# yuanqing-wang/stag

Hardware: AMD Instinct MI355X
Metric: aggregated edges/sec, stochastic-aggregation layer-forward, ogbn-arxiv-shaped CSR (higher is better)
Workload: dtype f32

## Files before the change

stag_amd/csrc/agg_kernel.hpp:

```cpp
#pragma once
#include "../../include/stag_hip.h"
#include "noise.hpp"
#include "entry_args.hpp"
#include <stdlib.h>

namespace stag {

struct AggArgs {
  const int32_t* indptr;
  const int32_t* indices;
  const int32_t* eid;
  const int32_t* nidx;
  int32_t n_rows;
  const float* x;
  int64_t ldx;
  int32_t D;
  uint32_t ldxb;
  uint32_t ldwb;
  uint32_t x_bytes;
  int32_t wide;
  const float* p0;
  const float* p1;
  float p0s, p1s;
  int32_t pmode;
  int32_t nflags, in_norm;
  int32_t wgroup;
  PhiloxKey key;
  uint32_t pos_lo, pos_hi;
  uint32_t chunk_base;
  int32_t n_heavy;
  int32_t n_heavy_blocks;
  struct alignas(32) Walk {
    int32_t smask, sshift;
    int32_t jh_heavy;
    int32_t jh_light;
    int32_t sh;
    int32_t lbase;
    int32_t sl;
    int32_t n_total;
  } walk;
  const int32_t* xcd;
  const float* src_scale;
  const float* dst_scale;
  int32_t mean;
  float* out;
  float* outx[3];
  int32_t mc;
  uint64_t mc_stride;
  int64_t ldo;
  float* norm_scale_out;
  const float* xown;
  int64_t ldxo;
  const float* own_scale;
  float* eg0;
  float* eg1;
  float* dp_part;
  const stag_unit* units;
  const stag_unit* units_plan;
  int32_t n_units;
  const int32_t* long_rows;
  const int32_t* long_seg_ptr;
  int32_t n_long;
  int32_t n_seg;
  int32_t* seg_counters;
  float* ws;
  int32_t ws_stride;
  uint32_t ws_bytes;
  uint32_t idx_bytes;
};

__device__ __forceinline__ void load4(const float* p, int k0, int D, bool vec, float (&v)[4]) {
  if (vec) {
    const float4 t = *reinterpret_cast<const float4*>(p + k0);
    v[0] = t.x; v[1] = t.y; v[2] = t.z; v[3] = t.w;
  } else {
#pragma unroll
    for (int j = 0; j < 4; ++j) v[j] = (k0 + j < D) ? p[k0 + j] : 0.0f;
  }
}

__device__ __forceinline__ void store4(float* p, int k0, int D, bool vec, const float (&v)[4]) {
  if (vec) {
    *reinterpret_cast<float4*>(p + k0) = make_float4(v[0], v[1], v[2], v[3]);
  } else {
#pragma unroll
    for (int j = 0; j < 4; ++j)
      if (k0 + j < D) p[k0 + j] = v[j];
  }
}

__device__ __forceinline__ void store4_sc1(__amdgpu_buffer_rsrc_t rsrc, uint32_t off, int k0, int D,
                                           bool vec, const float (&v)[4]) {
  typedef unsigned int u32x4 __attribute__((ext_vector_type(4)));
  if (vec) {
    const u32x4 t = {__float_as_uint(v[0]), __float_as_uint(v[1]), __float_as_uint(v[2]),
                     __float_as_uint(v[3])};
    __builtin_amdgcn_raw_buffer_store_b128(t, rsrc, (int)off, 0, 16);
  } else {
#pragma unroll
    for (int j = 0; j < 4; ++j)
      if (k0 + j < D)
        __builtin_amdgcn_raw_buffer_store_b32(__float_as_uint(v[j]), rsrc, (int)(off + 4u * j), 0, 16);
  }
}

template <int NF, bool VEC>
__device__ __forceinline__ void kahan_sum_partials(const float* ws, int ws_stride, int s0, int s1,
                                                   int k0, int D, float (&sum)[4], float (&comp)[4]) {
  comp[0] = comp[1] = comp[2] = comp[3] = 0.f;
  sum[0] = sum[1] = sum[2] = sum[3] = 0.f;
#pragma unroll 1
  for (int s = s0; s < s1; s += NF) {
    float t[NF][4];
#pragma unroll
    for (int i = 0; i < NF; ++i) {
      if (s + i < s1) load4(ws + (int64_t)(s + i) * ws_stride, k0, D, VEC, t[i]);
      else t[i][0] = t[i][1] = t[i][2] = t[i][3] = 0.f;
    }
#pragma unroll
    for (int i = 0; i < NF; ++i)
#pragma unroll
      for (int q = 0; q < 4; ++q) {
        const float y = t[i][q] - comp[q];
        const float n = sum[q] + y;
        comp[q] = (n - sum[q]) - y;
        sum[q] = n;
      }
  }
}

__device__ __forceinline__ void agg_epilogue_extra(const AggArgs& a, float* out, int v, int deg, int k0,
                                                   bool vec, float (&acc)[4]);

constexpr int kCombineGroup = 16;
template <int NF, bool VEC, int LPE, int SLOTS>
__device__ __forceinline__ void two_level_sum(const float* ws, int ws_stride, int s0, int s1, int k0,
                                              int D, int sl, int slot0, float (&sum)[4]) {
  float comp[4] = {0.f, 0.f, 0.f, 0.f};
  sum[0] = sum[1] = sum[2] = sum[3] = 0.f;
#pragma unroll 1
  for (int g0 = s0; g0 < s1; g0 += kCombineGroup * SLOTS) {
    const int gs = g0 + sl * kCombineGroup;
    float gsum[4] = {0.f, 0.f, 0.f, 0.f}, gres[4] = {0.f, 0.f, 0.f, 0.f};
    if (gs < s1) {
      const int ge = min(gs + kCombineGroup, s1);
      kahan_sum_partials<NF, VEC>(ws, ws_stride, gs, ge, k0, D, gsum, gres);
    }
#pragma unroll
    for (int j = 0; j < SLOTS; ++j) {
      if (g0 + j * kCombineGroup < s1) {
#pragma unroll
        for (int q = 0; q < 4; ++q) {
          const float gj = SLOTS > 1 ? __int_as_float(__builtin_amdgcn_ds_bpermute(
                                           slot0 + j * (LPE << 2), __float_as_int(gsum[q])))
                                     : gsum[q];
          const float rj = SLOTS > 1 ? __int_as_float(__builtin_amdgcn_ds_bpermute(
                                           slot0 + j * (LPE << 2), __float_as_int(gres[q])))
                                     : gres[q];
          comp[q] += rj;
          const float y = gj - comp[q];
          const float n = sum[q] + y;
          comp[q] = (n - sum[q]) - y;
          sum[q] = n;
        }
      }
    }
  }
#pragma unroll
  for (int q = 0; q < 4; ++q) sum[q] -= comp[q];
}

__device__ __forceinline__ void agg_epilogue_to(const AggArgs& a, float* out, float* norm_scale_out, int v, int deg,
                                                int k0, bool vec, float (&acc)[4], const float (&wsum)[4]);
__device__ __forceinline__ void agg_epilogue(const AggArgs& a, int v, int deg, int k0, bool vec,
                                             float (&acc)[4], const float (&wsum)[4]) {
  agg_epilogue_to(a, a.out, a.norm_scale_out, v, deg, k0, vec, acc, wsum);
}
__device__ __forceinline__ void agg_epilogue_to(const AggArgs& a, float* out, float* norm_scale_out, int v, int deg,
                                                int k0, bool vec, float (&acc)[4], const float (&wsum)[4]) {
  float dv = a.dst_scale ? a.dst_scale[v] : 1.0f;
  if (a.mean) dv *= __builtin_amdgcn_rcpf((float)(deg > 1 ? deg : 1));
  if (a.in_norm) {
    float s[4];
#pragma unroll
    for (int j = 0; j < 4; ++j) {
      s[j] = (wsum[j] != 0.0f) ? (float)deg / wsum[j] : 1.0f;
      acc[j] *= s[j];
    }
    if (norm_scale_out) store4(norm_scale_out + (int64_t)v * a.D, k0, a.D, vec, s);
  }
  if (!out) return;
#pragma unroll
  for (int j = 0; j < 4; ++j) acc[j] *= dv;
  store4(out + (int64_t)v * a.ldo, k0, a.D, vec, acc);
}

__device__ __forceinline__ void agg_epilogue_extra(const AggArgs& a, float* out, int v, int deg, int k0,
                                                   bool vec, float (&acc)[4]) {
  float dv = a.dst_scale ? a.dst_scale[v] : 1.0f;
  if (a.mean) dv *= __builtin_amdgcn_rcpf((float)(deg > 1 ? deg : 1));
#pragma unroll
  for (int j = 0; j < 4; ++j) acc[j] *= dv;
  store4(out + (int64_t)v * a.ldo, k0, a.D, vec, acc);
}

__device__ __forceinline__ const float* row_at(const float* base, int idx, uint32_t stride_bytes,
                                               uint32_t koff, bool wide) {
  const char* b = reinterpret_cast<const char*>(base);
  if (wide) return reinterpret_cast<const float*>(b + (uint64_t)(uint32_t)idx * stride_bytes + koff);
  return reinterpret_cast<const float*>(b + (__umul24((uint32_t)idx, stride_bytes) + koff));
}

typedef unsigned int u32x4_t __attribute__((ext_vector_type(4)));
__device__ __forceinline__ void bufrow4(__amdgpu_buffer_rsrc_t rsrc, int idx, uint32_t stride_bytes,
                                        uint32_t koff, float (&v)[4]) {
#ifndef STAG_X_AUX
#define STAG_X_AUX 0
#endif
  const u32x4_t t = __builtin_amdgcn_raw_buffer_load_b128(
      rsrc, (int)(__umul24((uint32_t)idx, stride_bytes) + koff), 0, STAG_X_AUX);
  v[0] = __uint_as_float(t.x); v[1] = __uint_as_float(t.y);
  v[2] = __uint_as_float(t.z); v[3] = __uint_as_float(t.w);
}

__device__ __forceinline__ void loadrow4(const float* p, int k0, int D, bool vec, float (&v)[4]) {
  if (vec) {
    const float4 t = *reinterpret_cast<const float4*>(p);
    v[0] = t.x; v[1] = t.y; v[2] = t.z; v[3] = t.w;
  } else {
#pragma unroll
    for (int j = 0; j < 4; ++j) v[j] = (k0 + j < D) ? p[j] : 0.0f;
  }
}

#ifndef STAG_KAHAN_MIN_LEN
#define STAG_KAHAN_MIN_LEN 16
#endif
constexpr int kKahanMinLen = STAG_KAHAN_MIN_LEN;

#ifndef STAG_BLK_RNG
#define STAG_BLK_RNG 2
#endif
#ifndef STAG_BLK_MEM
#define STAG_BLK_MEM 2
#endif
#ifndef STAG_WAVES_PER_SIMD
#define STAG_WAVES_PER_SIMD 1
#endif
#ifndef STAG_BLOCK_THREADS
#define STAG_BLOCK_THREADS 256
#endif
#ifndef STAG_LOAD_PRIO
#define STAG_LOAD_PRIO 1
#endif
#ifndef STAG_PRIO_MIN_LEN
#define STAG_PRIO_MIN_LEN 24
// ... 498 lines not shown
      __builtin_amdgcn_s_setprio(3);
#endif
      T.fetch_idx(I, p0);
      T.pin_idx(I);
      T.fetch_rows(R, I, p0);
#if STAG_LOAD_PRIO
      if (len > STAG_PRIO_MIN_LEN) __builtin_amdgcn_s_setprio(2); else __builtin_amdgcn_s_setprio(0);
#endif
      T.compute(R, I, p0);
    }
    }
  }

#ifdef STAG_TRACE
  if (trace) trace[1] = wall_clock64();
#endif
  if constexpr (PEDGE == 4) {
#pragma unroll
    for (int i = 0; i < 2; ++i)
#pragma unroll
      for (int q = 0; q < 4; ++q) dp_out[i][q] = T.DP.v[i][q];
  }
  if (slot < 0) {
    if (sl != 0) return;
    agg_epilogue(a, v, len, k0, VEC, T.acc, T.wsum);
    if constexpr (NOUT > 1) {
#pragma unroll
      for (int o = 0; o < NOUT - 1; ++o) {
        if constexpr (WN) agg_epilogue_to(a, a.outx[o], nullptr, v, len, k0, VEC, T.X.acc[o], T.XW.w[o]);
        else agg_epilogue_extra(a, a.outx[o], v, len, k0, VEC, T.X.acc[o]);
      }
    }
#ifdef STAG_TRACE
    if (trace) trace[3] = wall_clock64();
#endif
    return;
  }
  const int r = v;
  const __amdgpu_buffer_rsrc_t rws = __builtin_amdgcn_make_buffer_rsrc(a.ws, 0, (int)a.ws_bytes, 0x00020000);
  const uint32_t woff = (uint32_t)slot * ((uint32_t)a.ws_stride * 4u) + (uint32_t)k0 * 4u;
  if (sl == 0) {
    store4_sc1(rws, woff, k0, a.D, VEC, T.acc);
    if (PEDGE != 3 && PEDGE != 4 && a.in_norm) store4_sc1(rws, woff + (uint32_t)(NOUT * a.D) * 4u, k0, a.D, VEC, T.wsum);
    if constexpr (NOUT > 1) {
#pragma unroll
      for (int o = 0; o < NOUT - 1; ++o) {
        store4_sc1(rws, woff + (uint32_t)(o + 1) * (uint32_t)a.D * 4u, k0, a.D, VEC, T.X.acc[o]);
        if constexpr (WN) store4_sc1(rws, woff + (uint32_t)(NOUT + o + 1) * (uint32_t)a.D * 4u, k0, a.D, VEC, T.XW.w[o]);
      }
    }
  }
  const int s0 = a.long_seg_ptr[r], s1 = a.long_seg_ptr[r + 1];
  asm volatile("s_waitcnt vmcnt(0)" ::: "memory");
  int ticket = 0;
  int32_t* counter = a.seg_counters + (int64_t)blockIdx.y * a.n_long + r;
  if (c == 0 && sl == 0)
    ticket = __hip_atomic_fetch_add(counter, 1, __ATOMIC_RELAXED, __HIP_MEMORY_SCOPE_AGENT);
  const int lane0 = ((int)(threadIdx.x & 63) - c - sl * LPE) << 2;
  ticket = __builtin_amdgcn_ds_bpermute(lane0, ticket);
#ifdef STAG_TRACE
  if (trace) trace[2] = wall_clock64();
#endif
  if (ticket != (s1 - s0) - 1) return;
  __builtin_amdgcn_fence(__ATOMIC_ACQUIRE, "agent");
  asm volatile("s_waitcnt vmcnt(0)" ::: "memory");
  if (c == 0 && sl == 0) *counter = 0;
  const int row = a.long_rows[r];
  const int deg = a.indptr[row + 1] - a.indptr[row];
#ifndef STAG_COMBINE_NF
#define STAG_COMBINE_NF 8
#endif
  constexpr int NF = STAG_COMBINE_NF;
  float facc[4], fws[4] = {0.f, 0.f, 0.f, 0.f};
  const int slot0 = lane0 + (c << 2);
  two_level_sum<NF, VEC, LPE, SLOTS>(a.ws, a.ws_stride, s0, s1, k0, a.D, sl, slot0, facc);
  if (PEDGE != 3 && PEDGE != 4 && a.in_norm) two_level_sum<NF, VEC, LPE, SLOTS>(a.ws + NOUT * a.D, a.ws_stride, s0, s1, k0, a.D, sl, slot0, fws);
  if (sl != 0) return;
  agg_epilogue(a, row, deg, k0, VEC, facc, fws);
#pragma unroll
  for (int o = 0; o < NOUT - 1; ++o) {
    two_level_sum<NF, VEC, LPE, SLOTS>(a.ws + (o + 1) * a.D, a.ws_stride, s0, s1, k0, a.D, sl, slot0, facc);
    if constexpr (WN) {
      two_level_sum<NF, VEC, LPE, SLOTS>(a.ws + (NOUT + o + 1) * a.D, a.ws_stride, s0, s1, k0, a.D, sl, slot0, fws);
      agg_epilogue_to(a, a.outx[o], nullptr, row, deg, k0, VEC, facc, fws);
    } else {
      agg_epilogue_extra(a, a.outx[o], row, deg, k0, VEC, facc);
    }
  }
#ifdef STAG_TRACE
  if (trace) trace[3] = wall_clock64();
#endif
}

template <int KIND, int LPE>
constexpr int mult_of() {
  constexpr bool RNG = KIND >= kNormal;
  return LPE <= 4 ? (RNG ? STAG_MULT_LPE4 : 2 * STAG_MULT_LPE4)
         : LPE == 8 ? (RNG ? STAG_MULT_LPE8 : 4 * STAG_MULT_LPE8)
         : LPE == 16 ? (RNG ? STAG_MULT_LPE16 : 2 * STAG_MULT_LPE16)
                     : STAG_MULT_WIDE;
}
#ifndef STAG_HSLOTS_LPE4
#define STAG_HSLOTS_LPE4 4
#endif
#ifndef STAG_HSLOTS_LPE8
#define STAG_HSLOTS_LPE8 4
#endif
#ifndef STAG_HSLOTS_LPE16
#define STAG_HSLOTS_LPE16 2
#endif
#ifndef STAG_HSLOTS_LPE32
// ... 107 lines not shown
#ifndef STAG_MULT_WALK_WIDE
#define STAG_MULT_WALK_WIDE 2
#endif
    constexpr int MULT_W = NOUT != 1 ? 1 : (KIND == kNone && PEDGE == 0 && LPE >= 64) ? STAG_MULT_WALK_WIDE : mult_of<KIND, LPE>();
    agg_unit<KIND, LPE, VEC, PEDGE, 1, MULT_W, NOUT, MC, WN, true>(a, unit, c, 0);
  }
}

template <int KIND, int LPE, bool VEC>
__global__ __launch_bounds__(STAG_BLOCK_THREADS, STAG_WAVES_PER_SIMD) void agg_dp_kernel(const AggArgs a) {
  constexpr int TEAMS = STAG_BLOCK_THREADS / LPE;
  __shared__ float s_dp[TEAMS][2][LPE * 4];
  const int c = threadIdx.x % LPE, tm = threadIdx.x / LPE;
  const int unit = blockIdx.x * TEAMS + tm;
  float dp[2][4] = {{0.f, 0.f, 0.f, 0.f}, {0.f, 0.f, 0.f, 0.f}};
  if (unit < a.n_units) agg_unit<KIND, LPE, VEC, 4, 1, 1>(a, unit, c, 0, dp);
#pragma unroll
  for (int i = 0; i < 2; ++i)
#pragma unroll
    for (int q = 0; q < 4; ++q) s_dp[tm][i][c * 4 + q] = dp[i][q];
  __syncthreads();
  float* part = a.dp_part + ((int64_t)blockIdx.y * gridDim.x + blockIdx.x) * (2 * LPE * 4);
  for (int i = threadIdx.x; i < 2 * LPE * 4; i += STAG_BLOCK_THREADS) {
    float sum = 0.f;
#pragma unroll
    for (int j = 0; j < TEAMS; ++j) sum += s_dp[j][i / (LPE * 4)][i % (LPE * 4)];
    part[i] = sum;
  }
}

template <int KIND>
hipError_t agg_launch(const AggArgs& a, bool vec, hipStream_t stream);

#ifndef STAG_XCD_PLANLESS
#define STAG_XCD_PLANLESS 1
#endif
#ifndef STAG_AGG_LDS_BYTES
#define STAG_AGG_LDS_BYTES 0
#endif
inline bool plain_launch_ok(const AggArgs& a, bool vec, int pedge) {
  return vec && pedge == 0 && a.pmode == STAG_PARAM_SCALAR && !a.outx[0] && !a.dp_part && !a.mc && a.out &&
         !a.src_scale && !a.in_norm && !a.nidx && (a.nflags & ~(kFlagRelu | kFlagLogScale)) == 0 &&
         (a.wide & 1) == 0 && a.x_bytes != 0 && a.idx_bytes != 0;
}

template <int KIND>
void agg_launch_plain(const AggArgs& a, int lpe, bool walk, dim3 grid, hipStream_t s);

inline bool plain_enabled() {
#if defined(STAG_TRACE) || defined(STAG_EXP_NO_ROWS)
  return false;
#endif
  const char* e = getenv("STAG_AGG_PLAIN");
  return !(e && e[0] == '0' && e[1] == 0);
}

template <int KIND>
inline void agg_launch_small(const AggArgs& a_in, bool vec, int tiles, hipStream_t s) {
  AggArgs a = a_in;
  constexpr int LPE = 32, TPB = STAG_BLOCK_THREADS / LPE, TPBH = STAG_BLOCK_THREADS / (LPE * heavy_slots_of<KIND, LPE, true>());
  a.n_heavy_blocks = (a.n_heavy + TPBH - 1) / TPBH;
  const dim3 grid(a.n_heavy_blocks + (a.n_units - a.n_heavy + TPB - 1) / TPB, tiles), block(STAG_BLOCK_THREADS);
  if (grid.x == 0) return;
  if (vec) hipLaunchKernelGGL((agg_kernel<KIND, LPE, true, 0, 1, false, false, false, true>), grid, block, STAG_AGG_LDS_BYTES, s, a);
  else     hipLaunchKernelGGL((agg_kernel<KIND, LPE, false, 0, 1, false, false, false, true>), grid, block, STAG_AGG_LDS_BYTES, s, a);
}

template <int KIND, int LPE>
inline void agg_launch_shape(const AggArgs& a_in, bool vec, int pedge, int tiles, hipStream_t s) {
  if constexpr (LPE == 32 && heavy_slots_of<KIND, 32, true>() != heavy_slots_of<KIND, 32, false>()) {
    if (!a_in.outx[0] && !a_in.dp_part && pedge == 0 && !a_in.xcd && a_in.units && a_in.n_heavy > 0 &&
        a_in.n_units <= STAG_SMALL_UNITS) {
      agg_launch_small<KIND>(a_in, vec, tiles, s);
      return;
    }
  }
  AggArgs a = a_in;
  constexpr int TPB = STAG_BLOCK_THREADS / LPE;
  constexpr int HS = heavy_slots_of<KIND, LPE>();
  constexpr int TPBH = STAG_BLOCK_THREADS / (LPE * HS);
  const bool slotted = !(HS == 1 || a.outx[0] || pedge == 3 || a.dp_part);
  if (!slotted) a.n_heavy = 0;
  const bool plain = !a.outx[0] && !a.dp_part && pedge == 0;
  if (a.xcd && a.dp_part) { a.xcd = nullptr; a.units = a.units_plan; }
  a.n_heavy_blocks = (a.n_heavy + TPBH - 1) / TPBH;
  dim3 grid(a.n_heavy_blocks + (a.n_units - a.n_heavy + TPB - 1) / TPB, tiles);
  bool walk = false;
  AggArgs::Walk& w = a.walk;
  if (a.xcd) {
    walk = true;
    w.smask = STAG_XCD_STRIPES - 1; w.sshift = 3;
    w.jh_heavy = slotted ? (w.sh + TPBH - 1) / TPBH : 0;
    w.jh_light = slotted ? 0 : (w.sh + TPB - 1) / TPB;
    w.lbase = STAG_XCD_STRIPES * w.sh;
    w.n_total = STAG_XCD_STRIPES * (w.sh + w.sl);
    grid.x = STAG_XCD_STRIPES * (w.jh_heavy + w.jh_light + (w.sl + TPB - 1) / TPB);
  } else if (STAG_XCD_PLANLESS && !a.dp_part && !a.units && a.n_units >= STAG_XCD_STRIPES * TPB && a.n_units < (1 << 30)) {
    walk = true;
    w = AggArgs::Walk{STAG_XCD_STRIPES - 1, 3, 0, 0, 0, 0, 0, a.n_units};
    w.sl = ((a.n_units + STAG_XCD_STRIPES - 1) / STAG_XCD_STRIPES + TPB - 1) / TPB * TPB;
    grid.x = STAG_XCD_STRIPES * (w.sl / TPB);
  } else if (!plain && !a.dp_part) {
    walk = true;
    w = AggArgs::Walk{0, 0, 0, 0, a.n_heavy, a.n_heavy, a.n_units - a.n_heavy, a.n_units};
    w.jh_heavy = slotted ? a.n_heavy_blocks : 0;
    w.jh_light = slotted ? 0 : (w.sh + TPB - 1) / TPB;
// ... 15 lines not shown
    if (a.mc && a.outx[0]) {
      if (vec) hipLaunchKernelGGL((agg_kernel<KIND, LPE, true, 0, 2, true, false, true>), grid, block, STAG_AGG_LDS_BYTES, s, a);
      else     hipLaunchKernelGGL((agg_kernel<KIND, LPE, false, 0, 2, true, false, true>), grid, block, STAG_AGG_LDS_BYTES, s, a);
      return;
    }
  }
  if constexpr (KIND == kNormal || KIND == kUniform) {
    if (a.outx[0]) {
      if (vec) hipLaunchKernelGGL((agg_kernel<KIND, LPE, true, 0, 3, false, false, true>), grid, block, STAG_AGG_LDS_BYTES, s, a);
      else     hipLaunchKernelGGL((agg_kernel<KIND, LPE, false, 0, 3, false, false, true>), grid, block, STAG_AGG_LDS_BYTES, s, a);
      return;
    }
  }
  if constexpr (KIND == kNormal || KIND == kUniform) {
    if (a.dp_part) {
      if (vec) hipLaunchKernelGGL((agg_dp_kernel<KIND, LPE, true>), grid, block, STAG_AGG_LDS_BYTES, s, a);
      else     hipLaunchKernelGGL((agg_dp_kernel<KIND, LPE, false>), grid, block, STAG_AGG_LDS_BYTES, s, a);
      return;
    }
    if (pedge == 3) {
      if (vec) hipLaunchKernelGGL((agg_kernel<KIND, LPE, true, 3, 1, false, false, true>), grid, block, STAG_AGG_LDS_BYTES, s, a);
      else     hipLaunchKernelGGL((agg_kernel<KIND, LPE, false, 3, 1, false, false, true>), grid, block, STAG_AGG_LDS_BYTES, s, a);
      return;
    }
  }
  if constexpr (KIND >= kNormal) {
    if (pedge == 1) {
      if (vec) hipLaunchKernelGGL((agg_kernel<KIND, LPE, true, 1, 1, false, false, true>), grid, block, STAG_AGG_LDS_BYTES, s, a);
      else     hipLaunchKernelGGL((agg_kernel<KIND, LPE, false, 1, 1, false, false, true>), grid, block, STAG_AGG_LDS_BYTES, s, a);
      return;
    }
    if (pedge == 2) {
      if (vec) hipLaunchKernelGGL((agg_kernel<KIND, LPE, true, 2, 1, false, false, true>), grid, block, STAG_AGG_LDS_BYTES, s, a);
      else     hipLaunchKernelGGL((agg_kernel<KIND, LPE, false, 2, 1, false, false, true>), grid, block, STAG_AGG_LDS_BYTES, s, a);
      return;
    }
  }
  if constexpr (KIND >= kNormal && (LPE == 32 || LPE == 64)) {
    if (plain_launch_ok(a, vec, pedge) && plain_enabled()) {
      agg_launch_plain<KIND>(a, LPE, walk, grid, s);
      return;
    }
  }
  if (walk) {
    if (vec) hipLaunchKernelGGL((agg_kernel<KIND, LPE, true, 0, 1, false, false, true>), grid, block, STAG_AGG_LDS_BYTES, s, a);
    else     hipLaunchKernelGGL((agg_kernel<KIND, LPE, false, 0, 1, false, false, true>), grid, block, STAG_AGG_LDS_BYTES, s, a);
    return;
  }
  if (vec) hipLaunchKernelGGL((agg_kernel<KIND, LPE, true, 0>), grid, block, STAG_AGG_LDS_BYTES, s, a);
  else     hipLaunchKernelGGL((agg_kernel<KIND, LPE, false, 0>), grid, block, STAG_AGG_LDS_BYTES, s, a);
}

template <int KIND>
inline hipError_t agg_launch_impl(const AggArgs& a, bool vec, hipStream_t s) {
  const int nchunk = (a.D + 3) / 4;
  const int pedge = (KIND < kNormal) ? 0 : a.pmode == STAG_PARAM_PER_EDGE1 ? (a.eg0 ? 3 : 1)
                    : a.pmode == STAG_PARAM_PER_EDGE ? 2 : 0;
  const int lpe = lanes_for(nchunk, 1);
  const int tiles = (nchunk + lpe - 1) / lpe;
  switch (lpe) {
    case 64: agg_launch_shape<KIND, 64>(a, vec, pedge, tiles, s); break;
    case 32: agg_launch_shape<KIND, 32>(a, vec, pedge, tiles, s); break;
    case 16: agg_launch_shape<KIND, 16>(a, vec, pedge, tiles, s); break;
    case 8:  agg_launch_shape<KIND, 8>(a, vec, pedge, tiles, s); break;
    case 4:  agg_launch_shape<KIND, 4>(a, vec, pedge, tiles, s); break;
    case 2:  agg_launch_shape<KIND, 2>(a, vec, pedge, tiles, s); break;
    default: agg_launch_shape<KIND, 1>(a, vec, pedge, tiles, s); break;
  }
  return hipGetLastError();
}

}
```

stag_amd/csrc/api.hip:

```cpp
#include <algorithm>
#include <cmath>
#include <cstring>
#include <vector>

#include "../../include/stag_hip.h"
#include "agg_kernel.hpp"
#include "agg_max.hpp"
#include "entry_args.hpp"

using namespace stag;

namespace stag {
template <int KIND>
hipError_t agg_launch(const AggArgs& a, bool vec, hipStream_t stream);
}

namespace {

__global__ void philox_raw_kernel(PhiloxKey key, int64_t pos0, int64_t n_pos, int n_chunk,
                                  uint32_t* out) {
  const int64_t i = (int64_t)blockIdx.x * blockDim.x + threadIdx.x;
  if (i >= n_pos * n_chunk) return;
  uint32_t r[4];
  philox_at(pos0 + i / n_chunk, (uint32_t)(i % n_chunk), key, r);
// ... 765 lines not shown
    for (int f = 0; f < fine; ++f) {
      const int32_t lo = start[(size_t)x * fine + f], hi = start[(size_t)x * fine + f + 1];
      int32_t first = lo, edges = 0, units = 0;
      for (int32_t p = lo; p < hi; ++p) {
        const int32_t len = units_host[order[p]].len;
        if (units > 0 && (edges + len > max_edges || units == max_units)) {
          batches[x].emplace_back(first, units);
          first = p; edges = 0; units = 0;
        }
        edges += len; ++units;
      }
      if (units > 0) batches[x].emplace_back(first, units);
    }
  size_t per = 0;
  for (auto& b : batches) per = std::max(per, b.size());
  const int64_t nb = (int64_t)per * STAG_XCD_STRIPES;
  if (nb > 0x7FFFFFFFll) return STAG_EINVAL;
  *n_blocks_out = (int32_t)nb;
  if (!units_out_host) return STAG_OK;
  int32_t at = 0;
  block_ptr_host[0] = 0;
  for (size_t j = 0; j < per; ++j)
    for (int x = 0; x < STAG_XCD_STRIPES; ++x) {
      if (j < batches[x].size())
        for (int32_t p = 0; p < batches[x][j].second; ++p) units_out_host[at++] = units_host[order[(size_t)batches[x][j].first + p]];
      block_ptr_host[j * STAG_XCD_STRIPES + x + 1] = at;
    }
  return STAG_OK;
}
}
}

int stag_plan_blocks_xcd(const stag_unit* units_host, int32_t n_units, int64_t n_edges, int32_t fine, int32_t max_edges,
                         int32_t max_units, stag_unit* units_out_host, int32_t* block_ptr_host, int32_t* n_blocks_out) {
  if (n_units < 0 || n_edges < 0 || fine < 1 || fine > STAG_XCD_FINE_MAX || max_edges <= 0 || max_units <= 0 ||
      !n_blocks_out || (n_units > 0 && !units_host) || ((units_out_host == nullptr) != (block_ptr_host == nullptr)))
    return STAG_EINVAL;
  return plan_blocks_xcd_impl(units_host, n_units, fine, XcdKeyByPosition{n_edges > 0 ? n_edges : 1, STAG_XCD_STRIPES * fine},
                              max_edges, max_units, units_out_host, block_ptr_host, n_blocks_out);
}

int stag_plan_blocks_xcd_ranges(const stag_unit* units_host, int32_t n_units, const int64_t* cuts_host,
                                const int32_t* keys_host, int32_t n_ranges, int32_t fine, int32_t max_edges, int32_t max_units,
                                stag_unit* units_out_host, int32_t* block_ptr_host, int32_t* n_blocks_out) {
  if (n_units < 0 || fine < 1 || fine > STAG_XCD_FINE_MAX || max_edges <= 0 || max_units <= 0 || !n_blocks_out ||
      (n_units > 0 && !units_host) || ((units_out_host == nullptr) != (block_ptr_host == nullptr)) ||
      !xcd_ranges_ok(cuts_host, keys_host, n_ranges, fine)) return STAG_EINVAL;
  return plan_blocks_xcd_impl(units_host, n_units, fine, XcdKeyByRange{cuts_host, keys_host, n_ranges}, max_edges, max_units,
                              units_out_host, block_ptr_host, n_blocks_out);
}

size_t stag_plan_workspace_bytes(int32_t n_seg, int32_t D, int32_t in_norm) {
  if (n_seg <= 0 || D <= 0) return 0;
  return (size_t)n_seg * (size_t)D * (in_norm ? 2u : 1u) * sizeof(float);
}

int stag_philox_raw(uint64_t seed, uint64_t offset, int64_t pos0, int64_t n_pos, int32_t n_chunk,
                    uint32_t* out, void* stream) {
  if (!out || n_pos < 0 || n_chunk <= 0 || !aligned16(out)) return STAG_EINVAL;
  const int64_t n = n_pos * n_chunk;
  if (n == 0) return STAG_OK;
  hipLaunchKernelGGL(philox_raw_kernel, dim3((unsigned)((n + 255) / 256)), dim3(256), 0,
                     (hipStream_t)stream, make_key(seed, offset, nullptr), pos0, n_pos, n_chunk, out);
  return hipGetLastError() == hipSuccess ? STAG_OK : STAG_EIO;
}

int stag_normal_tables(float* rad, float* cosv, float* sinv, void* stream) {
  if (!rad || !cosv || !sinv) return STAG_EINVAL;
  hipLaunchKernelGGL(normal_tables_kernel, dim3((1u << 23) / 256), dim3(256), 0, (hipStream_t)stream, rad, cosv, sinv);
  return hipGetLastError() == hipSuccess ? STAG_OK : STAG_EIO;
}

struct EdgeGradOut {
  const float* xown;
  int64_t ldxo;
  float* eg0;
  float* eg1;
  float* dp_part;
};
static int agg_common(const stag_csr* csr, const stag_plan* plan, const float* x, int64_t ldx,
                      int32_t D, const stag_noise_spec* spec, int32_t reduce, const float* src_scale,
                      const float* dst_scale, float* out, int64_t ldo, float* norm_scale_out,
                      int nout, float* const* extra, int mc, uint64_t mc_stride, void* stream,
                      const EdgeGradOut* eg = nullptr) {
  int rc = check_csr(csr);
  if (rc) return rc;
  rc = check_spec(spec, csr->n_edges, D);
  if (rc) return rc;
  if (D <= 0 || (ldx != 0 && ldx < D) || ldo < D) return STAG_EINVAL;
  if (reduce != STAG_REDUCE_SUM && reduce != STAG_REDUCE_MEAN) return STAG_EINVAL;
  if (csr->n_dst == 0) return STAG_OK;
  if (!out && !norm_scale_out && !eg) return STAG_EINVAL;
  if (csr->n_edges > 0 && !x) return STAG_EINVAL;

  AggArgs a{};
  a.indptr = csr->indptr; a.indices = csr->indices; a.eid = csr->eid; a.nidx = csr->nidx;
  a.n_rows = csr->n_dst;
  a.x = x; a.ldx = ldx; a.D = D;
  a.ldxb = (uint32_t)(ldx * 4); a.ldwb = (uint32_t)D * 4u;
  {
    const uint64_t xbytes = (uint64_t)csr->n_src * (uint64_t)ldx * 4u;
    const uint64_t wbytes = (uint64_t)csr->n_edges * (uint64_t)D * 4u;
    const bool x_narrow = xbytes < (1ull << 32) && csr->n_src < (1 << 24) && (uint64_t)ldx * 4u < (1u << 24);
    const bool w_narrow = wbytes < (1ull << 32) && csr->n_edges < (1 << 24) && (uint64_t)D * 4u < (1u << 24);
    a.wide = (x_narrow ? 0 : 1) | (w_narrow ? 0 : 2);
    a.x_bytes = x_narrow ? (uint32_t)(ldx == 0 ? (uint64_t)D * 4u : xbytes) : 0u;
    a.idx_bytes = csr->n_edges < (1 << 30) ? (uint32_t)csr->n_edges * 4u : 0u;
  }
  fill_spec(a, spec, spec->deriv);
  a.in_norm = spec->in_norm;
  a.wgroup = (spec->kind == STAG_NOISE_EXPLICIT && spec->group > 1) ? spec->group : 1;
  if (a.wgroup > 1 && (D % a.wgroup != 0 || spec->in_norm)) return STAG_EINVAL;
  rc = check_positions(spec, csr->n_edges, D, spec->kind >= STAG_NOISE_NORMAL);
  if (rc) return rc;
  a.src_scale = src_scale; a.dst_scale = dst_scale; a.mean = (reduce == STAG_REDUCE_MEAN);
  a.out = out; a.ldo = ldo; a.norm_scale_out = norm_scale_out;
  for (int o = 0; o + 1 < nout; ++o) a.outx[o] = extra[o];
  a.mc = mc; a.mc_stride = mc_stride;
  if (eg) {
    a.xown = eg->xown; a.ldxo = eg->ldxo; a.own_scale = dst_scale; a.eg0 = eg->eg0; a.eg1 = eg->eg1;
    a.dp_part = eg->dp_part;
  }

  const bool use_plan = plan_in_use(plan);
  const bool has_segs = use_plan && plan->n_seg > 0;
  const bool xcd = use_plan && plan->xcd_order && !(eg && eg->dp_part);
  const size_t need = has_segs ? stag_plan_workspace_bytes(plan->n_seg, nout * D, spec->in_norm) : 0;
  rc = check_plan(plan, kPlanHeavy | (xcd ? kPlanXcd : 0) | kPlanSegPtr | kPlanWorkspace | kPlanNarrow | kPlanCounters, need);
  if (rc) return rc;
  fill_plan(a, csr, plan);
  if (use_plan) {
    a.units_plan = plan->units;
    a.n_heavy = plan->n_heavy;
    if (xcd) {
      a.xcd = plan->xcd_order;
      a.units = xcd_units(plan);
      a.walk.sh = plan->xcd_stride_heavy;
      a.walk.sl = plan->xcd_stride_light;
    }
  }
  if (has_segs) {
    a.ws_stride = D * nout * (spec->in_norm ? 2 : 1); a.ws_bytes = (uint32_t)need;
    a.seg_counters = plan->seg_counters; a.n_seg = plan->n_seg;
  }

  bool vec = (D % 4 == 0) && (ldx % 4 == 0) && (ldo % 4 == 0) && aligned16(x) && (!out || aligned16(out));
  if (norm_scale_out) vec = vec && aligned16(norm_scale_out);
  for (int o = 0; o + 1 < nout; ++o) vec = vec && aligned16(extra[o]);
  if (spec->kind == STAG_NOISE_EXPLICIT) vec = vec && aligned16(spec->p0);
  if (spec->kind >= STAG_NOISE_NORMAL && spec->param_mode != STAG_PARAM_SCALAR &&
      spec->param_mode != STAG_PARAM_PER_EDGE1)
    vec = vec && aligned16(spec->p0) && (!spec->p1 || aligned16(spec->p1));
  if (has_segs) vec = vec && aligned16(plan->workspace);
  if (eg && eg->xown) vec = vec && aligned16(eg->xown) && (eg->ldxo % 4 == 0);

  hipStream_t s = (hipStream_t)stream;
  auto launch = [&](const AggArgs& args) -> hipError_t {
    switch (spec->kind) {
      case STAG_NOISE_NONE: return agg_launch<kNone>(args, vec, s);
      case STAG_NOISE_EXPLICIT: return agg_launch<kExplicit>(args, vec, s);
      case STAG_NOISE_NORMAL: return agg_launch<kNormal>(args, vec, s);
      case STAG_NOISE_UNIFORM: return agg_launch<kUniform>(args, vec, s);
      default: return agg_launch<kBernoulli>(args, vec, s);
    }
  };
  if (launch(a) != hipSuccess) return STAG_EIO;
  return STAG_OK;
}

int stag_agg_fwd(const stag_csr* csr, const stag_plan* plan, const float* x, int64_t ldx,
                 int32_t D, const stag_noise_spec* spec, int32_t reduce, const float* src_scale,
                 const float* dst_scale, float* out, int64_t ldo, float* norm_scale_out,
                 void* stream) {
  return agg_common(csr, plan, x, ldx, D, spec, reduce, src_scale, dst_scale, out, ldo, norm_scale_out,
                    1, nullptr, 0, 0, stream);
}

int stag_agg_fwd_mc(const stag_csr* csr, const stag_plan* plan, const float* x, int64_t ldx,
                    int32_t D, const stag_noise_spec* spec, int32_t n_samples, int64_t offset_stride,
                    int32_t reduce, const float* src_scale, const float* dst_scale, float* out,
                    int64_t ldo, int64_t sample_stride, void* stream) {
  if (!spec || n_samples < 1 || offset_stride < 0 || !out) return STAG_EINVAL;
  if (spec->kind < STAG_NOISE_NORMAL || spec->deriv) return STAG_EINVAL;
  if (spec->param_mode != STAG_PARAM_SCALAR && spec->param_mode != STAG_PARAM_PER_CHANNEL) return STAG_EINVAL;
  if (n_samples > 1 && sample_stride < (int64_t)(csr ? csr->n_dst : 0) * ldo) return STAG_EINVAL;
  stag_noise_spec sp = *spec;
  const int kmax = spec->in_norm ? 2 : 4;
  for (int32_t s0 = 0; s0 < n_samples;) {
    const int k = (n_samples - s0 >= 4 && kmax >= 4) ? 4 : (n_samples - s0 >= 2) ? 2 : 1;
    sp.offset = spec->offset + (uint64_t)s0 * (uint64_t)offset_stride;
    float* extra[3] = {nullptr, nullptr, nullptr};
    for (int o = 1; o < k; ++o) extra[o - 1] = out + (int64_t)(s0 + o) * sample_stride;
    const int rc = agg_common(csr, plan, x, ldx, D, &sp, reduce, src_scale, dst_scale,
                              out + (int64_t)s0 * sample_stride, ldo, nullptr, k, extra, k > 1 ? 1 : 0,
                              (uint64_t)offset_stride, stream);
    if (rc) return rc;
// ... 425 lines not shown
```

stag_amd/ops.py:

```python
import ctypes as C

import torch

from . import _lib, _torch_ext
from .graph import DEFAULT_SEG_LEN
from .noise import EdgeNoise
from .random import _MASK64

_REDUCE = {"sum": _lib.REDUCE_SUM, "mean": _lib.REDUCE_MEAN}


def _owner(graph):
    return graph._cache_owner() if hasattr(graph, "_cache_owner") else graph


def _f32c(t):
    if t is None:
        return None
    if t.dtype != torch.float32:
        t = t.float()
    return t.contiguous()


def _none_spec():
    if _torch_ext.available():
        return _NONE_ARGS
    s = _lib.NoiseSpec()
    s.kind = _lib.NOISE_NONE
    return s


def _explicit_spec(w, relu=False, in_norm=False, group=0):
    if _torch_ext.available():
        return ([_lib.NOISE_EXPLICIT, 0, int(relu), int(in_norm), 0, int(group), 0, 0], [0, 0, 0], [0.0, 0.0], w, None, None)
    s = _lib.NoiseSpec()
    s.kind = _lib.NOISE_EXPLICIT
    s.p0 = w.data_ptr()
    s.relu, s.in_norm, s.group = int(relu), int(in_norm), int(group)
    return s


def _noise_spec(noise, in_norm=None):
    if _torch_ext.available():
        return noise.torch_args(in_norm=in_norm)
    s = noise.spec()
    if in_norm is not None:
        s.in_norm = int(in_norm)
    return s


def _targs_or_c(spec):
    return _targs_to_ctypes(spec) if isinstance(spec, tuple) else spec


def _spec_in_norm(spec):
    return bool(spec[0][3]) if isinstance(spec, tuple) else bool(spec.in_norm)


def _plan_struct(csrv, seg_len, tiles, nbytes, dev, plan_t=None, width=None, gat_width=None, drawn=False):
    if plan_t is None:
        plan_t = csrv.plan(seg_len)
    if plan_t is None:
        return None, None
    ws = torch.empty(nbytes // 4, dtype=torch.float32, device=dev) if nbytes else None
    key = (tiles, _lib.stream_of(dev))
    counters = plan_t["counters"].get(key)
    if counters is None:
        counters = torch.zeros(max(plan_t["n_long"], 1) * tiles, dtype=torch.int32, device=dev)
        plan_t["counters"][key] = counters
    order, strides, fine = csrv.xcd_order(plan_t, width, drawn) if width and plan_t.get("xcd_on") else (None, (0, 0), 0)
    units, block_ptr, n_blocks = plan_t["units"], plan_t["block_ptr"], plan_t["n_blocks"]
    if gat_width and plan_t.get("xcd_on"):
        blocks = csrv.gat_blocks(plan_t, gat_width)
        if blocks is not None:
            units, block_ptr, n_blocks, fine = blocks[0], blocks[1], blocks[2], -blocks[3]
            order = units
    plan_c = plan_t.setdefault("_structs", {}).get(key + (fine,))
    if plan_c is None:
        plan_c = _lib.Plan(plan_t["seg_len"], plan_t["n_units"], plan_t["n_long"], plan_t["n_seg"],
                           _lib.ptr(units), _lib.ptr(plan_t["long_rows"]),
                           _lib.ptr(plan_t["long_seg_ptr"]), _lib.ptr(counters), None, 0,
                           plan_t["n_heavy"] if units is plan_t["units"] else 0, n_blocks, _lib.ptr(block_ptr),
                           _lib.ptr(order), *strides)
        plan_t["_structs"][key + (fine,)] = plan_c
    plan_c.workspace, plan_c.workspace_bytes = _lib.ptr(ws), nbytes
    return plan_c, (ws, counters)


_NONE_ARGS = ([_lib.NOISE_NONE, 0, 0, 0, 0, 0, 0, 0], [0, 0, 0], [0.0, 0.0], None, None, None)


def _plan_args(csrv, plan_t, tiles, dev, width=None, drawn=False):
    if plan_t is None:
        return (None, None, None, None, None, None, [0, 0, 0, 0, 0, 0, 0, 0])
    key = (tiles, _lib.stream_of(dev))
    counters = plan_t["counters"].get(key)
    if counters is None:
        counters = torch.zeros(max(plan_t["n_long"], 1) * tiles, dtype=torch.int32, device=dev)
        plan_t["counters"][key] = counters
    order, strides, _ = csrv.xcd_order(plan_t, width, drawn) if width and plan_t.get("xcd_on") else (None, (0, 0), 0)
    ints = [plan_t["seg_len"], plan_t["n_units"], plan_t["n_long"], plan_t["n_seg"], plan_t["n_heavy"], plan_t["n_blocks"],
            *strides]
    return (plan_t["units"], plan_t["long_rows"], plan_t["long_seg_ptr"], plan_t["block_ptr"], order, counters, ints)


def _agg_fwd_torch(csrv, x, noise_args, reduce, src_scale, dst_scale, seg_len, want_norm_scale, broadcast_x):
    dev = _lib.require_device(x, csrv.indptr, src_scale, dst_scale)
    D = x.numel() if broadcast_x else x.shape[1]
    plan_t = csrv.plan(seg_len)
    out, ns = torch.ops.stag.agg_fwd(*csrv.torch_args(), *_plan_args(csrv, plan_t, (D + 255) // 256, dev, width=D,
                                                                     drawn=noise_args[0][0] >= _lib.NOISE_NORMAL), x,
                                     broadcast_x, *noise_args, reduce, src_scale, dst_scale, want_norm_scale)
    return out, (ns if want_norm_scale else None)


def _agg_raw(csrv, x, D, spec, reduce, src_scale, dst_scale, seg_len, want_norm_scale=False,
             broadcast_x=False, out=None, plan_t=None, ns_out=None):
    if isinstance(spec, tuple):
        if out is None and plan_t is None:
            return _agg_fwd_torch(csrv, x, spec, reduce, src_scale, dst_scale, seg_len, want_norm_scale, broadcast_x)
        spec = _targs_to_ctypes(spec)
    dev = _lib.require_device(x, csrv.indptr, src_scale, dst_scale)
    if out is None:
        out = torch.empty((csrv.n_dst, D), dtype=torch.float32, device=dev)
    ns = ns_out if ns_out is not None else (
        torch.empty((csrv.n_dst, D), dtype=torch.float32, device=dev) if want_norm_scale else None)
    if csrv.n_dst == 0:
        return out, ns
    if plan_t is None:
        plan_t = csrv.plan(seg_len)
    nbytes = (_lib.lib().stag_plan_workspace_bytes(plan_t["n_seg"], D, int(spec.in_norm))
              if plan_t is not None else 0)
    plan_c, _keep = _plan_struct(csrv, seg_len, (D + 255) // 256, nbytes, dev, plan_t, width=D,
                                 drawn=spec.kind >= _lib.NOISE_NORMAL)
    cs = csrv.struct()
    with _lib.on_device(dev):
        rc = _lib.lib().stag_agg_fwd(
            C.byref(cs), C.byref(plan_c) if plan_c is not None else None, _lib.ptr(x),
            0 if broadcast_x else x.stride(0), D, C.byref(spec), reduce, _lib.ptr(src_scale),
            _lib.ptr(dst_scale), _lib.ptr(out), D, _lib.ptr(ns), _lib.stream_of(dev))
    _lib.check(rc, "stag_agg_fwd")
    return out, ns


_HALF_DTYPES = {torch.float16: _lib.DTYPE_F16, torch.bfloat16: _lib.DTYPE_BF16}


def _agg_half_raw(csrv, x, D, spec, reduce, src_scale, dst_scale, seg_len, plan_t=None):
    spec = _targs_or_c(spec)
    dev = _lib.require_device(x, csrv.indptr, src_scale, dst_scale)
    out = torch.empty((csrv.n_dst, D), dtype=torch.float32, device=dev)
    if csrv.n_dst == 0:
# ... 1387 lines not shown
                            if (want_dp and ctx.needs_input_grad[10 + i]) else None)
            return (torch.zeros_like(el) if ctx.needs_input_grad[0] else None,
                    torch.zeros_like(er) if ctx.needs_input_grad[1] else None,
                    torch.zeros_like(ft) if ctx.needs_input_grad[2] else None,
                    torch.zeros_like(w) if want_dw else None, None, None, None, None, None, None, zp(0), zp(1))
        spec_tensors = ((noise.p0, noise.p1, noise.epoch) if noise is not None else (w, None, None))
        fused = _gat_bwd_fused(csrv, csrt, el, er, ft, stats, G, out, H, F, ctx.neg_slope, spec, nscale,
                               want_dw, ctx.seg_len, dev, ctx.attn_drop, want_dp=want_dp, spec_tensors=spec_tensors)
        if fused is not None:
            d_el, d_er, d_ft, dw = fused[:4]
            dps = [None, None]
            if want_dp:
                for i in range(2):
                    if ctx.needs_input_grad[10 + i]:
                        d, shape = fused[4 + i], ctx.pshapes[i]
                        dps[i] = d.sum().reshape(shape) if len(shape) == 0 or d.numel() != int(torch.Size(shape).numel()) else d.reshape(shape)
            return (d_el if ctx.needs_input_grad[0] else None, d_er if ctx.needs_input_grad[1] else None,
                    d_ft if ctx.needs_input_grad[2] else None, dw, None, None, None, None, None, None, dps[0], dps[1])
        if want_dp:
            raise NotImplementedError("vi=True GAT parameter gradients need the one-gather backward (stag_gat_bwd_dp)")
        if ctx.attn_drop is not None:
            raise NotImplementedError("attention dropout needs the one-gather GAT backward (stag_gat_bwd)")
        de = torch.empty((csrv.n_edges, H), dtype=torch.float32, device=dev)
        dw = torch.empty((csrv.n_edges, H), dtype=torch.float32, device=dev) if want_dw else None
        attn = (torch.empty((csrv.n_edges, H), dtype=torch.float32, device=dev)
                if ctx.needs_input_grad[2] else None)
        plan_c, _keep = _plan_struct(csrv, ctx.seg_len, 1, 0, dev)
        cs = csrv.struct()
        with _lib.on_device(dev):
            rc = _lib.lib().stag_gat_bwd_edge(
                C.byref(cs), C.byref(plan_c) if plan_c is not None else None, _lib.ptr(el),
                _lib.ptr(er), _lib.ptr(ft), _lib.ptr(stats), _lib.ptr(G), _lib.ptr(out), H, F,
                ctx.neg_slope, C.byref(spec), _lib.ptr(nscale), _lib.ptr(de), _lib.ptr(dw),
                _lib.ptr(attn), _lib.stream_of(dev))
        if rc == -38:
            raise NotImplementedError("GAT backward needs out_feats % 4 == 0 and out_feats / 4 a power of two")
        _lib.check(rc, "stag_gat_bwd_edge")
        ones = torch.ones(1, H, dtype=torch.float32, device=dev)
        d_el = d_er = d_ft = None
        if ctx.needs_input_grad[1]:
            d_er, _ = _agg_raw(csrv, ones, H, _explicit_spec(de), _lib.REDUCE_SUM, None, None,
                               ctx.seg_len, broadcast_x=True)
        if ctx.needs_input_grad[0]:
            d_el, _ = _agg_raw(csrt, ones, H, _explicit_spec(de), _lib.REDUCE_SUM, None, None,
                               ctx.seg_len, broadcast_x=True)
        if ctx.needs_input_grad[2]:
            d_ft, _ = _agg_raw(csrt, G.reshape(-1, HF), HF, _explicit_spec(attn, group=F), _lib.REDUCE_SUM, None, None,
                               ctx.seg_len)
            d_ft = d_ft.reshape(-1, H, F)
        return d_el, d_er, d_ft, dw, None, None, None, None, None, None, None, None


def _gat_plan_args(csrv, plan_t, dev, gat_width, transposed=False):
    key = (1, _lib.stream_of(dev))
    counters = plan_t["counters"].get(key)
    if counters is None:
        counters = torch.zeros(max(plan_t["n_long"], 1), dtype=torch.int32, device=dev)
        plan_t["counters"][key] = counters
    units, block_ptr, n_blocks, n_heavy = plan_t["units"], plan_t["block_ptr"], plan_t["n_blocks"], plan_t["n_heavy"]
    local = None
    if plan_t.get("xcd_on"):
        blocks = csrv.gat_blocks(plan_t, gat_width)
        if blocks is not None:
            units, block_ptr, n_blocks, n_heavy = blocks[0], blocks[1], blocks[2], 0
            local = units
    ints = [plan_t["seg_len"], plan_t["n_units"], plan_t["n_long"], plan_t["n_seg"], n_heavy, n_blocks, 0, 0]
    if transposed:
        return (units, plan_t["long_rows"], plan_t["long_seg_ptr"], block_ptr, counters, ints)
    return (units, plan_t["long_rows"], plan_t["long_seg_ptr"], block_ptr, local, counters, ints)


def _gat_drop_args(attn_drop):
    if attn_drop is None:
        return [], [], None
    s64 = lambda v: v - (1 << 64) if v >= (1 << 63) else v
    seed, off = int(attn_drop[1]) & ((1 << 64) - 1), int(attn_drop[2]) & ((1 << 64) - 1)
    return [1.0 - float(attn_drop[0])], [s64(seed), s64(off)], (attn_drop[3] if len(attn_drop) > 3 else None)


def _ctypes_to_targs(s, tensors):
    s64 = lambda v: v - (1 << 64) if v >= (1 << 63) else v
    p0, p1, epoch = tensors
    return ([s.kind, s.param_mode, s.relu, s.in_norm, s.deriv, s.group, s.chunk_base, s.p1_log],
            [s64(s.seed), s64(s.offset), s.pos_base], [s.p0_scalar, s.p1_scalar], p0, p1, epoch)


def _gat_bwd_fused(csrv, csrt, el, er, ft, stats, G, out, H, F, neg_slope, spec, nscale, want_dw, seg_len, dev,
                   attn_drop=None, want_dp=False, spec_tensors=(None, None, None)):
    lph = F // 4
    E = csrv.n_edges
    one = _GAT_BWD_ONE_GATHER or attn_drop is not None or want_dp
    if not (_GAT_BWD_FUSED and E > 0 and gat_cooperative_shape(H, F, seg_len)
            and (one or (lph & (lph - 1)) == 0)):
        return None
    if csrv.original_rows is not None:
        return _gat_bwd_reordered(csrv, csrt, el, er, ft, stats, G, out, H, F, neg_slope, _targs_or_c(spec), nscale, want_dw,
                                  seg_len, dev, attn_drop, want_dp)
    plan_f, plan_b = csrv.plan(seg_len, need=True), csrt.plan(seg_len, need=True)
    if _torch_ext.available() and not want_dp and (_GAT_BWD_ONE_GATHER or attn_drop is not None):
        if isinstance(spec, tuple):
            targs = spec
        else:
            targs = _ctypes_to_targs(spec, spec_tensors)
        try:
            d_el, d_er, d_ft, dw = torch.ops.stag.gat_bwd(
                *csrv.torch_args(), *_gat_plan_args(csrv, plan_f, dev, H * F),
                csrt.indptr, csrt.indices, csrt.eid, csrt.nidx, *_gat_plan_args(csrt, plan_b, dev, H * F, transposed=True),
                el, er, ft, stats, G, out, float(neg_slope), *targs, nscale, *_gat_drop_args(attn_drop), bool(want_dw))
        except RuntimeError as exc:
            if "rc=-38" in str(exc):
                return None
# ... 282 lines not shown
```

Measured before the change: 12.24 billion.

## Combine long-row segment partials hierarchically in groups before final fold

Long rows split across many segments are now reduced in two levels. The last segment of each group of kCombineGroup segments Kahan-sums that group's partials into a pair slot. The last group to finish then folds the group pairs and runs the epilogue. This replaces a single serial finisher summing every segment, and is meant to shorten the tail of very high-degree rows. In exchange it adds extra counters, workspace and a second atomic round, and it references kCombineGroup, which must be defined elsewhere.

```diff
diff --git a/stag_amd/csrc/agg_kernel.hpp b/stag_amd/csrc/agg_kernel.hpp
--- a/stag_amd/csrc/agg_kernel.hpp
+++ b/stag_amd/csrc/agg_kernel.hpp
@@ -67,6 +67,7 @@
   int32_t ws_stride;
   uint32_t ws_bytes;
   uint32_t idx_bytes;
+  int32_t combine_groups;
 };
 
 __device__ __forceinline__ void load4(const float* p, int k0, int D, bool vec, float (&v)[4]) {
@@ -170,6 +171,45 @@
   for (int q = 0; q < 4; ++q) sum[q] -= comp[q];
 }
 
+__host__ __device__ __forceinline__ int combine_pair_slot(int gs, int s0) { return 2 * (gs / kCombineGroup) + (gs == s0 ? 1 : 0); }
+__host__ __device__ __forceinline__ int combine_pair_slots(int n_seg) {
+  return n_seg > kCombineGroup ? 2 * ((n_seg - 1) / kCombineGroup) + 2 : 0;
+}
+template <int NP, bool VEC>
+__device__ __forceinline__ void fold_group_pairs(const float* pairs, int ws_stride, int s0, int s1, int k0, int D,
+                                                 float (&sum)[4]) {
+  float comp[4] = {0.f, 0.f, 0.f, 0.f};
+  sum[0] = sum[1] = sum[2] = sum[3] = 0.f;
+#pragma unroll 1
+  for (int g0 = s0; g0 < s1; g0 += kCombineGroup * NP) {
+    float t[NP][2][4];
+#pragma unroll
+    for (int i = 0; i < NP; ++i) {
+      const int gs = g0 + i * kCombineGroup;
+      if (gs < s1) {
+        const float* p = pairs + (int64_t)combine_pair_slot(gs, s0) * (2 * ws_stride);
+        load4(p, k0, D, VEC, t[i][0]);
+        load4(p + ws_stride, k0, D, VEC, t[i][1]);
+      }
+    }
+#pragma unroll
+    for (int i = 0; i < NP; ++i) {
+      if (g0 + i * kCombineGroup < s1) {
+#pragma unroll
+        for (int q = 0; q < 4; ++q) {
+          comp[q] += t[i][1][q];
+          const float y = t[i][0][q] - comp[q];
+          const float n = sum[q] + y;
+          comp[q] = (n - sum[q]) - y;
+          sum[q] = n;
+        }
+      }
+    }
+  }
+#pragma unroll
+  for (int q = 0; q < 4; ++q) sum[q] -= comp[q];
+}
+
 __device__ __forceinline__ void agg_epilogue_to(const AggArgs& a, float* out, float* norm_scale_out, int v, int deg,
                                                 int k0, bool vec, float (&acc)[4], const float (&wsum)[4]);
 __device__ __forceinline__ void agg_epilogue(const AggArgs& a, int v, int deg, int k0, bool vec,
@@ -202,6 +242,63 @@
 #pragma unroll
   for (int j = 0; j < 4; ++j) acc[j] *= dv;
   store4(out + (int64_t)v * a.ldo, k0, a.D, vec, acc);
+}
+
+#ifndef STAG_COMBINE_GROUP_NF
+#define STAG_COMBINE_GROUP_NF 8
+#endif
+template <bool VEC, int LPE, int PEDGE, int SLOTS, int NOUT, bool WN>
+__device__ __forceinline__ void combine_grouped(const AggArgs& a, __amdgpu_buffer_rsrc_t rws, int r, int slot, int s0,
+                                                int s1, int c, int sl, int k0, int lane0) {
+  constexpr int NG = STAG_COMBINE_GROUP_NF;
+  const int gs = s0 + (slot - s0) / kCombineGroup * kCombineGroup, ge = min(gs + kCombineGroup, s1);
+  int32_t* gcounter = a.seg_counters + a.combine_groups + (int64_t)blockIdx.y * a.n_seg + gs;
+  int ticket = 0;
+  if (c == 0 && sl == 0)
+    ticket = __hip_atomic_fetch_add(gcounter, 1, __ATOMIC_RELAXED, __HIP_MEMORY_SCOPE_AGENT);
+  ticket = __builtin_amdgcn_ds_bpermute(lane0, ticket);
+  if (ticket != (ge - gs) - 1) return;
+  if (SLOTS > 1 && sl != 0) return;
+  __builtin_amdgcn_fence(__ATOMIC_ACQUIRE, "agent");
+  asm volatile("s_waitcnt vmcnt(0)" ::: "memory");
+  if (c == 0) *gcounter = 0;
+  const int ncol = NOUT * ((PEDGE != 3 && PEDGE != 4 && a.in_norm) ? 2 : 1);
+  const uint32_t poff = (uint32_t)a.n_seg * ((uint32_t)a.ws_stride * 4u) +
+                        (uint32_t)combine_pair_slot(gs, s0) * ((uint32_t)a.ws_stride * 8u) + (uint32_t)k0 * 4u;
+#pragma unroll 1
+  for (int j = 0; j < ncol; ++j) {
+    float gsum[4], gres[4];
+    kahan_sum_partials<NG, VEC>(a.ws + j * a.D, a.ws_stride, gs, ge, k0, a.D, gsum, gres);
+    store4_sc1(rws, poff + (uint32_t)(j * a.D) * 4u, k0, a.D, VEC, gsum);
+    store4_sc1(rws, poff + (uint32_t)(a.ws_stride + j * a.D) * 4u, k0, a.D, VEC, gres);
+  }
+  asm volatile("s_waitcnt vmcnt(0)" ::: "memory");
+  int32_t* counter = a.seg_counters + (int64_t)blockIdx.y * a.n_long + r;
+  ticket = 0;
+  if (c == 0) ticket = __hip_atomic_fetch_add(counter, 1, __ATOMIC_RELAXED, __HIP_MEMORY_SCOPE_AGENT);
+  ticket = __builtin_amdgcn_ds_bpermute(lane0, ticket);
+  if (ticket != (s1 - s0 + kCombineGroup - 1) / kCombineGroup - 1) return;
+  __builtin_amdgcn_fence(__ATOMIC_ACQUIRE, "agent");
+  asm volatile("s_waitcnt vmcnt(0)" ::: "memory");
+  if (c == 0) *counter = 0;
+  const int row = a.long_rows[r];
+  const int deg = a.indptr[row + 1] - a.indptr[row];
+  const float* pairs = a.ws + (int64_t)a.n_seg * a.ws_stride;
+  float facc[4], fws[4] = {0.f, 0.f, 0.f, 0.f};
+  fold_group_pairs<NG / 2, VEC>(pairs, a.ws_stride, s0, s1, k0, a.D, facc);
+  if (PEDGE != 3 && PEDGE != 4 && a.in_norm) fold_group_pairs<NG / 2, VEC>(pairs + NOUT * a.D, a.ws_stride, s0, s1, k0, a.D, fws);
+  agg_epilogue(a, row, deg, k0, VEC, facc, fws);
+#pragma unroll
+  for (int o = 0; o < NOUT - 1; ++o) {
+    fold_group_pairs<NG / 2, VEC>(pairs + (o + 1) * a.D, a.ws_stride, s0, s1, k0, a.D, facc);
+    if constexpr (WN) {
+      fold_group_pairs<NG / 2, VEC>(pairs + (NOUT + o + 1) * a.D, a.ws_stride, s0, s1, k0, a.D, fws);
+      agg_epilogue_to(a, a.outx[o], nullptr, row, deg, k0, VEC, facc, fws);
+    } else {
+      agg_epilogue_extra(a, a.outx[o], row, deg, k0, VEC, facc);
+    }
+  }
+  asm volatile("; combine_grouped: done" ::: "memory");
 }
 
 __device__ __forceinline__ const float* row_at(const float* base, int idx, uint32_t stride_bytes,
@@ -806,11 +903,18 @@
   }
   const int s0 = a.long_seg_ptr[r], s1 = a.long_seg_ptr[r + 1];
   asm volatile("s_waitcnt vmcnt(0)" ::: "memory");
+  const int lane0 = ((int)(threadIdx.x & 63) - c - sl * LPE) << 2;
+  if (a.combine_groups && (s1 - s0) > kCombineGroup) {
+    combine_grouped<VEC, LPE, PEDGE, SLOTS, NOUT, WN>(a, rws, r, slot, s0, s1, c, sl, k0, lane0);
+#ifdef STAG_TRACE
+    if (trace) trace[2] = trace[3] = wall_clock64();
+#endif
+    return;
+  }
   int ticket = 0;
   int32_t* counter = a.seg_counters + (int64_t)blockIdx.y * a.n_long + r;
   if (c == 0 && sl == 0)
     ticket = __hip_atomic_fetch_add(counter, 1, __ATOMIC_RELAXED, __HIP_MEMORY_SCOPE_AGENT);
-  const int lane0 = ((int)(threadIdx.x & 63) - c - sl * LPE) << 2;
   ticket = __builtin_amdgcn_ds_bpermute(lane0, ticket);
 #ifdef STAG_TRACE
   if (trace) trace[2] = wall_clock64();
@@ -1024,6 +1128,11 @@
   return false;
 #endif
   const char* e = getenv("STAG_AGG_PLAIN");
+  return !(e && e[0] == '0' && e[1] == 0);
+}
+
+inline bool combine_groups_enabled() {
+  const char* e = getenv("STAG_COMBINE_GROUPS");
   return !(e && e[0] == '0' && e[1] == 0);
 }
 
@@ -1145,12 +1254,14 @@
 }
 
 template <int KIND>
-inline hipError_t agg_launch_impl(const AggArgs& a, bool vec, hipStream_t s) {
+inline hipError_t agg_launch_impl(const AggArgs& a_in, bool vec, hipStream_t s) {
+  AggArgs a = a_in;
   const int nchunk = (a.D + 3) / 4;
   const int pedge = (KIND < kNormal) ? 0 : a.pmode == STAG_PARAM_PER_EDGE1 ? (a.eg0 ? 3 : 1)
                     : a.pmode == STAG_PARAM_PER_EDGE ? 2 : 0;
   const int lpe = lanes_for(nchunk, 1);
   const int tiles = (nchunk + lpe - 1) / lpe;
+  if (a.combine_groups) a.combine_groups = tiles * a.n_long;
   switch (lpe) {
     case 64: agg_launch_shape<KIND, 64>(a, vec, pedge, tiles, s); break;
     case 32: agg_launch_shape<KIND, 32>(a, vec, pedge, tiles, s); break;
diff --git a/stag_amd/csrc/api.hip b/stag_amd/csrc/api.hip
--- a/stag_amd/csrc/api.hip
+++ b/stag_amd/csrc/api.hip
@@ -841,7 +841,8 @@
 
 size_t stag_plan_workspace_bytes(int32_t n_seg, int32_t D, int32_t in_norm) {
   if (n_seg <= 0 || D <= 0) return 0;
-  return (size_t)n_seg * (size_t)D * (in_norm ? 2u : 1u) * sizeof(float);
+  const size_t rows = (size_t)n_seg + 2u * (size_t)stag::combine_pair_slots(n_seg);
+  return rows * (size_t)D * (in_norm ? 2u : 1u) * sizeof(float);
 }
 
 int stag_philox_raw(uint64_t seed, uint64_t offset, int64_t pos0, int64_t n_pos, int32_t n_chunk,
@@ -931,6 +932,7 @@
   if (has_segs) {
     a.ws_stride = D * nout * (spec->in_norm ? 2 : 1); a.ws_bytes = (uint32_t)need;
     a.seg_counters = plan->seg_counters; a.n_seg = plan->n_seg;
+    a.combine_groups = combine_groups_enabled() ? 1 : 0;
   }
 
   bool vec = (D % 4 == 0) && (ldx % 4 == 0) && (ldo % 4 == 0) && aligned16(x) && (!out || aligned16(out));
diff --git a/stag_amd/ops.py b/stag_amd/ops.py
--- a/stag_amd/ops.py
+++ b/stag_amd/ops.py
@@ -57,17 +57,29 @@
     return bool(spec[0][3]) if isinstance(spec, tuple) else bool(spec.in_norm)
 
 
+_COMBINE_GROUP = 16
+
+
+def _counter_count(n_long, n_seg, tiles):
+    return max(n_long, 1) * tiles + (n_seg * tiles if n_seg > _COMBINE_GROUP else 0)
+
+
+def _plan_counters(plan_t, tiles, dev):
+    key = (tiles, _lib.stream_of(dev))
+    counters = plan_t["counters"].get(key)
+    if counters is None:
+        counters = torch.zeros(_counter_count(plan_t["n_long"], plan_t["n_seg"], tiles), dtype=torch.int32, device=dev)
+        plan_t["counters"][key] = counters
+    return key, counters
+
+
 def _plan_struct(csrv, seg_len, tiles, nbytes, dev, plan_t=None, width=None, gat_width=None, drawn=False):
     if plan_t is None:
         plan_t = csrv.plan(seg_len)
     if plan_t is None:
         return None, None
     ws = torch.empty(nbytes // 4, dtype=torch.float32, device=dev) if nbytes else None
-    key = (tiles, _lib.stream_of(dev))
-    counters = plan_t["counters"].get(key)
-    if counters is None:
-        counters = torch.zeros(max(plan_t["n_long"], 1) * tiles, dtype=torch.int32, device=dev)
-        plan_t["counters"][key] = counters
+    key, counters = _plan_counters(plan_t, tiles, dev)
     order, strides, fine = csrv.xcd_order(plan_t, width, drawn) if width and plan_t.get("xcd_on") else (None, (0, 0), 0)
     units, block_ptr, n_blocks = plan_t["units"], plan_t["block_ptr"], plan_t["n_blocks"]
     if gat_width and plan_t.get("xcd_on"):
@@ -93,11 +105,7 @@
 def _plan_args(csrv, plan_t, tiles, dev, width=None, drawn=False):
     if plan_t is None:
         return (None, None, None, None, None, None, [0, 0, 0, 0, 0, 0, 0, 0])
-    key = (tiles, _lib.stream_of(dev))
-    counters = plan_t["counters"].get(key)
-    if counters is None:
-        counters = torch.zeros(max(plan_t["n_long"], 1) * tiles, dtype=torch.int32, device=dev)
-        plan_t["counters"][key] = counters
+    _, counters = _plan_counters(plan_t, tiles, dev)
     order, strides, _ = csrv.xcd_order(plan_t, width, drawn) if width and plan_t.get("xcd_on") else (None, (0, 0), 0)
     ints = [plan_t["seg_len"], plan_t["n_units"], plan_t["n_long"], plan_t["n_seg"], plan_t["n_heavy"], plan_t["n_blocks"],
             *strides]
@@ -1591,11 +1599,7 @@
 
 
 def _gat_plan_args(csrv, plan_t, dev, gat_width, transposed=False):
-    key = (1, _lib.stream_of(dev))
-    counters = plan_t["counters"].get(key)
-    if counters is None:
-        counters = torch.zeros(max(plan_t["n_long"], 1), dtype=torch.int32, device=dev)
-        plan_t["counters"][key] = counters
+    _, counters = _plan_counters(plan_t, 1, dev)
     units, block_ptr, n_blocks, n_heavy = plan_t["units"], plan_t["block_ptr"], plan_t["n_blocks"], plan_t["n_heavy"]
     local = None
     if plan_t.get("xcd_on"):
```

Measured after the change: 12.58 billion, median of 6. 1.03x the previous value.
